# i2Nav-WHU/IC-GVINS

Hardware: AMD Instinct MI355X
Metric: frames/s at 1280x720, 300 feats, 10-KF window; residual/Jacobian eval/s (higher is better)
Workload: dtype u8/int64 front-end (f32/f64 solves), f64 factors

## Files before the change

ic-gvins_amd/csrc/detect.hip:

```cpp
#include <cfloat>

#include "icg_internal.h"


__device__ __forceinline__ unsigned int f32_order_key(float f) {
    unsigned int b = __float_as_uint(f);
    return (b & 0x80000000u) ? ~b : (b | 0x80000000u);
}
__device__ __forceinline__ float f32_from_order_key(unsigned int k) {
    unsigned int b = (k & 0x80000000u) ? (k & 0x7fffffffu) : ~k;
    return __uint_as_float(b);
}

#define FE_TW 60
#define FE_TH 16
#define FE_WAVES 4
#define FE_MAX_RADIUS 1022
#ifndef FE_RESIDENT_PER_XCD
#define FE_RESIDENT_PER_XCD 192
#endif

__device__ __forceinline__ float from_left(float v) {
    return __int_as_float(__builtin_amdgcn_mov_dpp(__float_as_int(v), 0x138, 0xF, 0xF, true));
}
__device__ __forceinline__ float from_right(float v) {
    return __int_as_float(__builtin_amdgcn_mov_dpp(__float_as_int(v), 0x130, 0xF, 0xF, true));
}

__device__ __forceinline__ unsigned int wave_or_to_lane63(unsigned int v) {
    v |= (unsigned int) __builtin_amdgcn_update_dpp(0, (int) v, 0xB1, 0xF, 0xF, false);
    v |= (unsigned int) __builtin_amdgcn_update_dpp(0, (int) v, 0x4E, 0xF, 0xF, false);
    v |= (unsigned int) __builtin_amdgcn_update_dpp(0, (int) v, 0x141, 0xF, 0xF, false);
    v |= (unsigned int) __builtin_amdgcn_update_dpp(0, (int) v, 0x140, 0xF, 0xF, false);
    v |= (unsigned int) __builtin_amdgcn_update_dpp(0, (int) v, 0x142, 0xA, 0xF, false);
    v |= (unsigned int) __builtin_amdgcn_update_dpp(0, (int) v, 0x143, 0xC, 0xF, false);
    return v;
}

#ifndef FE_CH
#define FE_CH 4
#endif
#define FE_GAP 6

__device__ __forceinline__ float fe_max(float a, float b) {
    float d;
    asm("v_max_f32 %0, %1, %2" : "=v"(d) : "v"(a), "v"(b));
    return d;
}

enum { FE_PLAIN = 0, FE_MIRRORS = 1, FE_PRIME = 2 };
struct fe_rows {
    int d0 = 0, d1 = 0, s0 = 0, s1 = 0;
    double hA0 = 0, hA1 = 0, hB0 = 0, hB1 = 0, hC0 = 0, hC1 = 0;
    float eC = 0.f, sideC = 0.f, m3T = 0.f, m3C = 0.f;
    bool unmC = false;
    float emax = -INFINITY;

    template <int MODE>
    __device__ __forceinline__ void chunk(unsigned int (&pix)[FE_CH], int y_last , const uint8_t *img,
                                          int base , int pitch, int ry, int h, unsigned int uc, int y0, int rh, int rw,
                                          unsigned int sel, float s, bool nms_col, int lane, int roi, int xcol, int32_t *cand_cnt,
                                          unsigned long long *cbase) {
        typedef unsigned int __attribute__((aligned(1))) u32u;
#pragma unroll
        for (int i = 0; i < FE_CH; i++) {
            const int y = y0 + i;
            const unsigned int v = __builtin_amdgcn_perm(0u, pix[i], sel);
            {
                const uint8_t *rowp = img + (size_t) icg_reflect1(min(max(ry + min(y + FE_CH, y_last), -1), h), h) * pitch;
                unsigned int vb = (unsigned int) base;
                asm("" : "+v"(vb));
                pix[i] = *reinterpret_cast<const u32u *>(rowp + vb);
            }
            const int a3 = (int) (v & 0xffu), b3 = (int) ((v >> 8) & 0xffu), c3 = (int) ((v >> 16) & 0xffu);
            const int dN = c3 - a3, sN = a3 + 2 * b3 + c3;
            if (MODE != FE_PRIME || i >= 2) {
                const int gxv = d0 + 2 * d1 + dN, gyv = sN - s0;
                const float dx = (float) gxv * s, dy = (float) gyv * s;
                const float cx = dx * dx, cm = dx * dy, cy = dy * dy;
                double hAn = ((double) from_left(cx) + (double) cx) + (double) from_right(cx);
                double hBn = ((double) from_left(cm) + (double) cm) + (double) from_right(cm);
                double hCn = ((double) from_left(cy) + (double) cy) + (double) from_right(cy);
                if (MODE != FE_PRIME) {
// ... 100 lines not shown
    }
    unsigned long long need;
    {
        unsigned int lo = (unsigned int) unmasked, hi = (unsigned int) (unmasked >> 32);
        lo = wave_or_to_lane63(lo);
        hi = wave_or_to_lane63(hi);
        need = ((unsigned long long) (unsigned int) __builtin_amdgcn_readlane((int) hi, 63) << 32) | (unsigned int) __builtin_amdgcn_readlane((int) lo, 63);
    }
    if (need == 0ull) return;
    typedef unsigned int __attribute__((aligned(1))) u32u;
    float emax = -INFINITY;
    while (need) {
        const int a = __ffsll((long long) need) - 1;
        unsigned long long closed = need;
#pragma unroll
        for (int g = 1; g <= FE_GAP; g++) closed |= need << g;
        const unsigned long long from_a = closed >> a;
        const int len                   = (~from_a == 0ull) ? 64 : __ffsll((long long) ~from_a) - 1;
        const unsigned long long runset = (len >= 64 ? ~0ull : ((1ull << len) - 1ull)) << a;
        const unsigned long long inrun  = need & runset;
        const int b                     = 63 - __builtin_clzll(inrun);
        need &= ~runset;
        const unsigned long long urun = (unmasked & inrun) >> a;
        const int y_first = by0 + a - 3, n_rows = b - a + 7;

        fe_rows st;
        st.emax = emax;
        unsigned int pix[FE_CH];
#pragma unroll
        for (int i = 0; i < FE_CH; i++) {
            const uint8_t *rowp = img + (size_t) icg_reflect1(min(max(R.ry + y_first + i, -1), h), h) * pitch;
            pix[i] = *reinterpret_cast<const u32u *>(rowp + (unsigned int) base);
        }
        const int y_last = y_first + n_rows - 1;
        st.chunk<FE_PRIME>(pix, y_last, img, base, pitch, R.ry, h, 0u, y_first, R.rh, R.rw, sel, s, nms_col, lane, roi, xcol, cand_cnt, cbase);
        for (int t0 = FE_CH; t0 < n_rows; t0 += FE_CH) {
            const unsigned int uc = t0 >= 5 ? (unsigned int) (urun >> (t0 - 5)) : (unsigned int) urun << (5 - t0);
            const int y0 = y_first + t0;
            if ((y0 <= 2 && 2 < y0 + FE_CH) || (y0 <= R.rh + 1 && R.rh + 1 < y0 + FE_CH))
                st.chunk<FE_MIRRORS>(pix, y_last, img, base, pitch, R.ry, h, uc, y0, R.rh, R.rw, sel, s, nms_col, lane, roi, xcol, cand_cnt, cbase);
            else
                st.chunk<FE_PLAIN>(pix, y_last, img, base, pitch, R.ry, h, uc, y0, R.rh, R.rw, sel, s, nms_col, lane, roi, xcol, cand_cnt, cbase);
        }
        emax = st.emax;
    }
    unsigned int key = emax == -INFINITY ? 0u : f32_order_key(emax);
#pragma unroll
    for (int m = 32; m >= 1; m >>= 1) {
        const unsigned int o = __shfl_xor(key, m, 64);
        key                  = o > key ? o : key;
    }
    if (lane == 0 && key) atomicMax(&roi_max[roi], key);
}

__global__ __launch_bounds__(64 * FE_WAVES) void k_min_eig_nms(const det_roi *rois, const uint8_t *frames, size_t slot_bytes,
                                                               const int32_t *slots, int pitch, int w, int h, const float2 *mask_pts,
                                                               const int32_t *mask_begin, const int32_t *mask_cnt , int radius,
                                                               const int32_t *vspan ,
                                                               unsigned int *roi_max,
                                                               unsigned long long *cand, size_t cand_plane, int32_t *cand_cnt,
                                                               int gx, int gy, int n_blocks, unsigned int m_roi, unsigned int m_gx) {
    __shared__ int vh[FE_MAX_RADIUS + 2];
    for (int a = threadIdx.x; a < radius + 2; a += 64 * FE_WAVES) vh[a] = vspan[a];
    __syncthreads();
    const int n_items = (n_blocks + FE_WAVES - 1) / FE_WAVES;
    const int chunk   = (n_items + 7) >> 3;
    const int x = blockIdx.x & 7, j = blockIdx.x >> 3, G = gridDim.x >> 3;
    const int wv  = __builtin_amdgcn_readfirstlane((int) (threadIdx.x >> 6));
    const int end = min((x + 1) * chunk, n_items);
    for (int it = x * chunk + j; it < end; it += G) {
        const int bl = it * FE_WAVES + wv;
        if (bl < n_blocks)
            fe_block(bl, vh, rois, frames, slot_bytes, slots, pitch, w, h, mask_pts, mask_begin, mask_cnt, radius, roi_max, cand, cand_plane, cand_cnt, gx, gy,
                     m_roi, m_gx);
    }
}

#define DET_MAX_PER_BLOCK 64

struct subpix_mask_t {
    float m[121];
};

struct subpix_smem {
    double terms[121][5];
    float patch[13][13];
    float cur[2];
    int stop;
};

#define DET_WAVE_SYNC()                                         \
    do {                                                        \
        __builtin_amdgcn_fence(__ATOMIC_SEQ_CST, "workgroup");  \
        __builtin_amdgcn_wave_barrier();                        \
    } while (0)

__device__ __forceinline__ float2 subpix_corner(subpix_smem &S, const det_roi &R, const uint8_t *img, int pitch, const float2 cT, int lane,
                                                const subpix_mask_t &M) {
    float cIx = cT.x, cIy = cT.y;
    int iter = 0;
    while (true) {
        const float ox = cIx - 6.f, oy = cIy - 6.f;
        const int iox = (int) floorf(ox), ioy = (int) floorf(oy);
        const float fa = ox - iox, fb = oy - ioy;
        const float w00 = (1.f - fa) * (1.f - fb), w01 = fa * (1.f - fb), w10 = (1.f - fa) * fb, w11 = fa * fb;
        for (int i = lane; i < 169; i += 64) {
            int r = i / 13, c = i - r * 13;
            int x0 = min(max(iox + c, 0), R.rw - 1), x1 = min(max(iox + c + 1, 0), R.rw - 1);
            int y0 = min(max(ioy + r, 0), R.rh - 1), y1 = min(max(ioy + r + 1, 0), R.rh - 1);
            const uint8_t *p0 = img + (size_t) (R.ry + y0) * pitch + R.rx;
            const uint8_t *p1 = img + (size_t) (R.ry + y1) * pitch + R.rx;
            float s00 = p0[x0], s01 = p0[x1], s10 = p1[x0], s11 = p1[x1];
            S.patch[r][c] = s00 * w00 + s01 * w01 + s10 * w10 + s11 * w11;
        }
        DET_WAVE_SYNC();
        for (int i = lane; i < 121; i += 64) {
            int r = i / 11, c = i - r * 11;
            double m   = M.m[i];
            double tgx = S.patch[r + 1][c + 2] - S.patch[r + 1][c];
            double tgy = S.patch[r + 2][c + 1] - S.patch[r][c + 1];
            double gxx = tgx * tgx * m, gxy = tgx * tgy * m, gyy = tgy * tgy * m;
            double px = c - 5, py = r - 5;
            S.terms[i][0] = gxx;
            S.terms[i][1] = gxy;
            S.terms[i][2] = gyy;
            S.terms[i][3] = gxx * px + gxy * py;
            S.terms[i][4] = gxy * px + gyy * py;
        }
        DET_WAVE_SYNC();
        double acc = 0;
        {
            const int q = lane % 5;
#pragma unroll 11
            for (int i = 0; i < 121; i++) acc += S.terms[i][q];
        }
        const double a = __shfl(acc, 0, 64), b = __shfl(acc, 1, 64), c = __shfl(acc, 2, 64);
        const double bb1 = __shfl(acc, 3, 64), bb2 = __shfl(acc, 4, 64);
        int st     = 0;
        float c2x = cIx, c2y = cIy;
        double det = a * c - b * b;
        if (fabs(det) <= DBL_EPSILON * DBL_EPSILON) {
            st = 1;
        } else {
            double scale = 1.0 / det;
            c2x          = (float) (cIx + c * scale * bb1 - b * scale * bb2);
            c2y          = (float) (cIy - b * scale * bb1 + a * scale * bb2);
            double err   = (double) ((c2x - cIx) * (c2x - cIx) + (c2y - cIy) * (c2y - cIy));
            if (c2x < 0 || c2x >= R.rw || c2y < 0 || c2y >= R.rh)
                st = 2;
            else if (!(iter + 1 < 20 && err > 0.01 * 0.01))
                st = 2;
        }
        if (st != 1) {
            cIx = c2x;
            cIy = c2y;
        }
        ++iter;
        DET_WAVE_SYNC();
        if (st) break;
    }
    if (fabsf(cIx - cT.x) > 5 || fabsf(cIy - cT.y) > 5) {
        cIx = cT.x;
        cIy = cT.y;
    }
    return make_float2(cIx, cIy);
}

__global__ __launch_bounds__(256) void k_select(const det_roi *rois, unsigned long long *cand, size_t cand_plane, int32_t *cand_cnt, unsigned int *roi_max,
                                                int min_dist, float2 *picks , int32_t *pick_cnt, int32_t *cnt_out, int max_pb) {
    __shared__ unsigned long long wbest[4];
    __shared__ unsigned long long best;
    const det_roi R = rois[blockIdx.x];
    const int t     = threadIdx.x;
    if (R.quota <= 0) {
        if (t == 0) pick_cnt[blockIdx.x] = 0, cnt_out[blockIdx.x] = 0;
        return;
    }
    unsigned long long *C = cand + (size_t) R.job * cand_plane + R.cand_base;
    const int n = cand_cnt[blockIdx.x];
    const double md2 = (double) min_dist * (double) min_dist;
    int quota = R.quota < max_pb ? R.quota : max_pb;
    int acc   = 0;
    {
        const unsigned int mk = roi_max[blockIdx.x];
        const double maxVal   = mk ? (double) f32_from_order_key(mk) : 0.0;
        const float thresh    = (float) (maxVal * 0.01);
        for (int i = t; i < n; i += 256)
            if (!(f32_from_order_key((unsigned int) (C[i] >> 32)) > thresh)) C[i] = 0;
        __syncthreads();
    }
    while (acc < quota) {
        unsigned long long k = 0;
        for (int i = t; i < n; i += 256) {
            unsigned long long c = C[i];
            k                    = c > k ? c : k;
        }
#pragma unroll
        for (int m = 32; m >= 1; m >>= 1) {
            unsigned long long o = __shfl_xor(k, m, 64);
            k                    = o > k ? o : k;
        }
        if ((t & 63) == 0) wbest[t >> 6] = k;
        __syncthreads();
        if (t == 0) {
            unsigned long long b = wbest[0];
            for (int i = 1; i < 4; i++) b = wbest[i] > b ? wbest[i] : b;
            best = b;
        }
        __syncthreads();
        const unsigned long long b = best;
        if (b == 0) break;
        const int idx = (int) (b & 0xffffffffu);
        const int by = idx / R.rw, bx = idx - by * R.rw;
        if (t == 0) picks[(size_t) blockIdx.x * max_pb + acc] = make_float2((float) bx, (float) by);
        acc++;
        if (min_dist >= 1) {
            for (int i = t; i < n; i += 256) {
                unsigned long long c = C[i];
                if (!c) continue;
                int ci = (int) (c & 0xffffffffu);
                int cy = ci / R.rw, cx = ci - cy * R.rw;
                float dx = (float) (cx - bx), dy = (float) (cy - by);
                if (c == b || (double) (dx * dx + dy * dy) < md2) C[i] = 0;
            }
        } else {
            for (int i = t; i < n; i += 256)
                if (C[i] == b) C[i] = 0;
        }
        __syncthreads();
    }
    if (t == 0) {
        pick_cnt[blockIdx.x] = acc;
        cnt_out[blockIdx.x]  = acc;
        roi_max[blockIdx.x]  = 0;
        cand_cnt[blockIdx.x] = 0;
    }
}

__global__ __launch_bounds__(64) void k_subpix(const det_roi *rois, const uint8_t *frames, size_t slot_bytes, const int32_t *slots, int pitch,
                                               const float2 *picks, float2 *corners_out, const int32_t *pick_cnt, int max_pb, subpix_mask_t M) {
    __shared__ subpix_smem SP;
    const int roi = blockIdx.x / max_pb, ci = blockIdx.x - roi * max_pb;
    if (ci >= pick_cnt[roi]) return;
    const det_roi R    = rois[roi];
    const uint8_t *img = frames + (size_t) slots[R.job] * slot_bytes;
    const float2 r     = subpix_corner(SP, R, img, pitch, picks[(size_t) roi * max_pb + ci], (int) threadIdx.x, M);
    if (threadIdx.x == 0) corners_out[(size_t) roi * max_pb + ci] = r;
}

static void circle_halfwidths(int radius, std::vector<int32_t> &hw) {
    hw.assign((size_t) radius + 1, -1);
    int err = 0, dx = radius, dy = 0, plus = 1, minus = (radius << 1) - 1;
    while (dx >= dy) {
        if (dx > hw[dy]) hw[dy] = dx;
        if (dy > hw[dx]) hw[dx] = dy;
        dy++;
        err += plus;
        plus += 2;
        int m = (err <= 0) - 1;
        err -= minus & m;
        dx += m;
        minus -= m & 2;
    }
}

static bool circle_row_spans(const std::vector<int32_t> &hw, std::vector<int32_t> &vh) {
    const int radius = (int) hw.size() - 1;
    vh.assign((size_t) radius + 2, -1);
    for (int a = 0; a <= radius; a++)
        for (int dy = 0; dy <= radius; dy++)
            if (hw[(size_t) dy] >= a) vh[(size_t) a] = dy;
    for (int a = 0; a <= radius; a++)
        for (int dy = 0; dy <= radius; dy++)
            if ((hw[(size_t) dy] >= a) != (dy <= vh[(size_t) a])) return false;
    return true;
}

static int ensure_roi_state(icg_ctx *ctx, int n_roi) {
    if (n_roi <= ctx->roi_state_cap) return 0;
    ICG_HIP(ctx, hipStreamSynchronize(ctx->stream));
    if (ctx->d_roi_max) (void) hipFree(ctx->d_roi_max);
    if (ctx->d_cand_cnt) (void) hipFree(ctx->d_cand_cnt);
    ctx->d_roi_max = nullptr, ctx->d_cand_cnt = nullptr, ctx->roi_state_cap = 0;
    const int cap = std::max(1024, 2 * n_roi);
    ICG_HIP(ctx, hipMalloc((void **) &ctx->d_roi_max, sizeof(uint32_t) * (size_t) cap));
    ICG_HIP(ctx, hipMalloc((void **) &ctx->d_cand_cnt, sizeof(int32_t) * (size_t) cap));
    ICG_HIP(ctx, hipMemsetAsync(ctx->d_roi_max, 0, sizeof(uint32_t) * (size_t) cap, ctx->stream));
    ICG_HIP(ctx, hipMemsetAsync(ctx->d_cand_cnt, 0, sizeof(int32_t) * (size_t) cap, ctx->stream));
    ctx->roi_state_cap = cap;
    return 0;
}

static subpix_mask_t subpix_window() {
    subpix_mask_t M;
    for (int i = 0; i < 11; i++) {
        float y  = (float) (i - 5) / 5;
        float vy = std::exp(-y * y);
        for (int j = 0; j < 11; j++) {
            float x         = (float) (j - 5) / 5;
            M.m[i * 11 + j] = (float) (vy * std::exp(-x * x));
        }
    }
    return M;
}

static int ensure_detect_ws(icg_ctx *ctx) {
    if (ctx->d_cand) return 0;
    const size_t w = ctx->cfg.width, h = ctx->cfg.height, nb = ctx->cfg.max_batch;
    ICG_HIP(ctx, hipMalloc((void **) &ctx->d_cand, sizeof(unsigned long long) * w * h * nb));
    return 0;
}

int icg_detect_check_grid(icg_ctx *ctx, const icg_detect_grid *grid) {
    if (grid->block_cols * grid->block_rows <= 0 || grid->block_w <= 6 || grid->block_h <= 6 || grid->block_cols * grid->block_w > ctx->cfg.width ||
        grid->block_rows * grid->block_h > ctx->cfg.height || grid->min_dist < 0 || grid->max_per_block <= 0 ||
        grid->max_per_block > DET_MAX_PER_BLOCK || grid->min_dist > FE_MAX_RADIUS)
        return icg_fail(ctx, ICG_ERR_INVALID, "bad detection grid");
    return 0;
}

static int detect_launch(icg_ctx *ctx, int n_roi, const icg_detect_grid *grid, const det_roi *d_rois, const int32_t *d_slots, const float2 *d_mask_pts,
                         const int32_t *d_mask_begin, const int32_t *d_mask_cnt, const int32_t *d_vh, float2 *d_picks, int32_t *d_pick_cnt,
                         float2 *d_corners, int32_t *d_corner_cnt) {
    const int w = ctx->cfg.width, h = ctx->cfg.height, pitch = ctx->lv[0].pitch, max_pb = grid->max_per_block;
    const size_t cand_plane = (size_t) w * h;
    {
        icg_prof_scope ps(ctx, "detect_min_eig_nms");
        const int gx = (grid->block_w + FE_TW - 1) / FE_TW, gy = (grid->block_h + FE_TH * FE_WAVES - 1) / (FE_TH * FE_WAVES);
        hipLaunchKernelGGL(k_min_eig_nms, dim3(std::min(icg_xcd_grid((gx * gy * n_roi + FE_WAVES - 1) / FE_WAVES), 8 * FE_RESIDENT_PER_XCD)), dim3(64 * FE_WAVES), 0, ctx->stream, d_rois, ctx->d_frames,
                           ctx->slot_bytes, d_slots, pitch, w, h, d_mask_pts, d_mask_begin, d_mask_cnt, grid->min_dist, d_vh, ctx->d_roi_max, ctx->d_cand,
                           cand_plane, ctx->d_cand_cnt, gx, gy, gx * gy * n_roi, icg_div_magic(gx * gy), icg_div_magic(gx));
    }
    {
        icg_prof_scope ps(ctx, "detect_select");
        hipLaunchKernelGGL(k_select, dim3(n_roi), dim3(256), 0, ctx->stream, d_rois, ctx->d_cand, cand_plane, ctx->d_cand_cnt, ctx->d_roi_max, grid->min_dist,
                           d_picks, d_pick_cnt, d_corner_cnt, max_pb);
    }
    {
        const subpix_mask_t M = subpix_window();
        icg_prof_scope ps(ctx, "detect_subpix");
        hipLaunchKernelGGL(k_subpix, dim3(n_roi * max_pb), dim3(64), 0, ctx->stream, d_rois, ctx->d_frames, ctx->slot_bytes, d_slots, pitch,
                           (const float2 *) d_picks, d_corners, (const int32_t *) d_pick_cnt, max_pb, M);
    }
    ICG_HIP(ctx, hipGetLastError());
    return ICG_OK;
}

extern "C" int icg_detect(icg_ctx *ctx, int n, const int32_t *slots, const icg_detect_grid *grid, const int32_t *mask_off,
                          const float *mask_pts, const int32_t *quota, int max_per_job, float *out_pts,
                          int32_t *out_count, int32_t *out_block) {
    if (!ctx || n < 0) return ICG_ERR_INVALID;
    if (n == 0) return ICG_OK;
    if (!slots || !grid || !mask_off || !quota || !out_pts || !out_count || max_per_job <= 0) return ICG_ERR_INVALID;
    if (n > ctx->cfg.max_batch) return icg_fail(ctx, ICG_ERR_CAPACITY, "detect batch %d > max_batch %d", n, ctx->cfg.max_batch);
    int rc = icg_detect_check_grid(ctx, grid);
    if (rc) return rc;
    const int nblk = grid->block_cols * grid->block_rows;
    for (int k = 0; k < n; k++)
        if (slots[k] < 0 || slots[k] >= ctx->cfg.n_slots) return icg_fail(ctx, ICG_ERR_INVALID, "bad slot");
    const int n_mask = mask_off[n];
    if (n_mask < 0 || (n_mask > 0 && !mask_pts)) return ICG_ERR_INVALID;
    ICG_HIP(ctx, hipSetDevice(ctx->cfg.device));
    if ((rc = ensure_detect_ws(ctx))) return rc;

    std::vector<det_roi> rois;
    for (int b = 0; b < n; b++)
        for (int k = 0; k < nblk; k++) {
            int q = quota[(size_t) b * nblk + k];
            if (q <= 0) continue;
            if (q > grid->max_per_block) q = grid->max_per_block;
            int cols = k % grid->block_cols, rows = k / grid->block_cols;
            det_roi R;
            R.job   = b;
            R.block = k;
            R.rx    = cols * grid->block_w;
            R.ry    = rows * grid->block_h;
            R.rw    = grid->block_w;
            R.rh    = grid->block_h;
            if (k != nblk - 1) {
                R.rw -= 5;
                R.rh -= 5;
            }
            R.quota     = q;
            R.cand_base = k * grid->block_w * grid->block_h;
            rois.push_back(R);
        }
    const int n_roi = (int) rois.size();
    for (int b = 0; b < n; b++) out_count[b] = 0;
    if (n_roi == 0) return ICG_OK;
    const int max_pb = grid->max_per_block;

    std::vector<int32_t> hw, vh;
    circle_halfwidths(grid->min_dist, hw);
    if (!circle_row_spans(hw, vh)) return icg_fail(ctx, ICG_ERR_INVALID, "circle span table of radius %d is not monotone", grid->min_dist);
    for (int b = 0; b < n; b++)
        if (mask_off[b] < 0 || mask_off[b] > mask_off[b + 1]) return icg_fail(ctx, ICG_ERR_INVALID, "mask_off is not non-decreasing");

    icg_call c(ctx);
    size_t need = sizeof(det_roi) * n_roi + sizeof(int32_t) * (2 * (size_t) n + 1 + vh.size()) + sizeof(float) * 2 * n_mask +
                  2 * (sizeof(float2) * max_pb + 16) * (size_t) n_roi + 8192;
    if ((rc = c.reserve(need))) return rc;
    const det_roi *d_rois  = c.in_zc(rois.data(), (size_t) n_roi);
    const int32_t *d_slots = c.in_zc(slots, (size_t) n);
    const int32_t *d_vh    = c.in(vh.data(), vh.size());
    const float2 *d_mpts   = (const float2 *) c.in(mask_pts, 2 * (size_t) n_mask);
    std::vector<int32_t> mcnt((size_t) n);
    for (int b = 0; b < n; b++) mcnt[(size_t) b] = mask_off[b + 1] - mask_off[b];
    const int32_t *d_moff  = c.in(mask_off, (size_t) n);
    const int32_t *d_mcnt  = c.in(mcnt.data(), (size_t) n);
    if ((rc = ensure_roi_state(ctx, n_roi))) return rc;
    if ((rc = c.seal())) return rc;
    std::vector<float> h_corners((size_t) n_roi * max_pb * 2);
    std::vector<int32_t> h_cnt((size_t) n_roi);
    float2 *d_picks = (float2 *) c.out((float *) nullptr, (size_t) n_roi * max_pb * 2);
    int32_t *d_pcnt = c.out((int32_t *) nullptr, (size_t) n_roi);
    float2 *z_corners  = (float2 *) c.out_zc(h_corners.data(), (size_t) n_roi * max_pb * 2);
    int32_t *z_cnt     = c.out_zc(h_cnt.data(), (size_t) n_roi);

    ICG_LAUNCH_GUARD(c);
    if ((rc = detect_launch(ctx, n_roi, grid, d_rois, d_slots, d_mpts, d_moff, d_mcnt, d_vh, d_picks, d_pcnt, z_corners, z_cnt))) return rc;
    if ((rc = c.finish())) return rc;

    for (int r = 0; r < n_roi; r++) {
        const det_roi &R = rois[r];
        for (int i = 0; i < h_cnt[r]; i++) {
// ... 31 lines not shown
```

ic-gvins_amd/csrc/lk.hip:

```cpp
#include <cfloat>

#include "dev_camera.h"
#include "icg_internal.h"

using namespace icgd;

#define LK_IT 24
#define LK_IS 28
#define LK_JT 32
#define LK_JS 36
#define LK_JM 5
#define LK_MAX_ITERS 30
#ifndef LK_WAVES_PER_EU
#define LK_WAVES_PER_EU 5
#endif

struct lk_smem {
    unsigned int I[LK_IT * LK_IS / 4];
    unsigned int J[LK_JT * LK_JS / 4 + 1];
};

__device__ __forceinline__ int dpp_add_xor1(int v) { return v + __builtin_amdgcn_update_dpp(0, v, 0xB1, 0xF, 0xF, false); }
__device__ __forceinline__ int dpp_add_xor2(int v) { return v + __builtin_amdgcn_update_dpp(0, v, 0x4E, 0xF, 0xF, false); }
__device__ __forceinline__ int dpp_add_half_mirror(int v) { return v + __builtin_amdgcn_update_dpp(0, v, 0x141, 0xF, 0xF, false); }
// ... 113 lines not shown
typedef unsigned int __attribute__((aligned(1))) lk_u32u;

__device__ __forceinline__ void lk_load_I(unsigned int (&v)[3], const unsigned char *I, int W, int H, int pitch, int ipx, int ipy,
                                          int lane) {
    const bool inside = ipx - 1 >= 0 && ipx - 1 + LK_IT <= W && ipy - 1 >= 0 && ipy - 1 + LK_IT <= H;
#pragma unroll
    for (int q = 0; q < 3; q++) {
        const int i = lane + 64 * q;
        const int r = i / 6, cd = i - r * 6;
        v[q] = 0;
        if (i < LK_IT * 6) {
            if (inside)
                v[q] = *reinterpret_cast<const lk_u32u *>(I + (size_t) (ipy - 1 + r) * pitch + (ipx - 1 + 4 * cd));
            else
                v[q] = lk_load4(I + (size_t) icg_reflect101(ipy - 1 + r, H) * pitch, ipx - 1 + 4 * cd, W);
        }
    }
}
__device__ __forceinline__ void lk_store_I(lk_smem &S, const unsigned int (&v)[3], int lane) {
#pragma unroll
    for (int q = 0; q < 3; q++) {
        const int i = lane + 64 * q;
        const int r = i / 6, cd = i - r * 6;
        if (i < LK_IT * 6) S.I[(r * LK_IS >> 2) + cd] = v[q];
    }
}
__device__ __forceinline__ void lk_load_J(unsigned int (&v)[4], const unsigned char *J, int W, int H, int pitch, int jx0, int jy0,
                                          int lane) {
    const int r = lane >> 1, c0 = (lane & 1) * 16;
    const bool inside = jx0 >= 0 && jx0 + LK_JT <= W && jy0 >= 0 && jy0 + LK_JT <= H;
    if (inside) {
        const unsigned char *row = J + (size_t) (jy0 + r) * pitch + (jx0 + c0);
#pragma unroll
        for (int q = 0; q < 4; q++) v[q] = *reinterpret_cast<const lk_u32u *>(row + 4 * q);
    } else {
        const unsigned char *row = J + (size_t) icg_reflect101(jy0 + r, H) * pitch;
#pragma unroll
        for (int q = 0; q < 4; q++) v[q] = lk_load4(row, jx0 + c0 + 4 * q, W);
    }
}
__device__ __forceinline__ void lk_store_J(lk_smem &S, const unsigned int (&v)[4], int lane) {
    const int r = lane >> 1, c0 = (lane & 1) * 16;
    unsigned int *dst = &S.J[(r * LK_JS + c0) >> 2];
#pragma unroll
    for (int q = 0; q < 4; q++) dst[q] = v[q];
}
__device__ __forceinline__ void lk_stage_J(lk_smem &S, const unsigned char *J, int W, int H, int pitch, int jx0, int jy0,
                                           int lane) {
    unsigned int v[4];
    lk_load_J(v, J, W, H, pitch, jx0, jy0, lane);
    lk_store_J(S, v, lane);
}

typedef short s16x2 __attribute__((ext_vector_type(2)));
typedef unsigned short u16x2 __attribute__((ext_vector_type(2)));

__device__ __forceinline__ unsigned int pk_add(unsigned int a, unsigned int b) {
    return __builtin_bit_cast(unsigned int, (u16x2) (__builtin_bit_cast(u16x2, a) + __builtin_bit_cast(u16x2, b)));
}
__device__ __forceinline__ unsigned int pk_sub(unsigned int a, unsigned int b) {
    return __builtin_bit_cast(unsigned int, (u16x2) (__builtin_bit_cast(u16x2, a) - __builtin_bit_cast(u16x2, b)));
}
__device__ __forceinline__ unsigned int pk_mul(unsigned int a, unsigned short k) {
    return __builtin_bit_cast(unsigned int, (u16x2) (__builtin_bit_cast(u16x2, a) * k));
}
__device__ __forceinline__ int dot2(unsigned int a, unsigned int b, int c) {
    return __builtin_amdgcn_sdot2(__builtin_bit_cast(s16x2, a), __builtin_bit_cast(s16x2, b), c, false);
}
__device__ __forceinline__ int dot2_keep(unsigned int a, unsigned int b, int c) {
    int d;
    asm("v_dot2_i32_i16 %0, %1, %2, %3" : "=v"(d) : "v"(a), "v"(b), "v"(c));
    return d;
}
__device__ __forceinline__ int dot2_keep_s(unsigned int a, unsigned int b, int c_uniform) {
    int d;
    asm("v_dot2_i32_i16 %0, %1, %2, %3" : "=v"(d) : "v"(a), "v"(b), "s"(c_uniform));
    return d;
}
__device__ __forceinline__ int dot2_zero(unsigned int a, unsigned int b) {
    int d;
    asm("v_dot2_i32_i16 %0, %1, %2, 0" : "=v"(d) : "v"(a), "v"(b));
    return d;
}
__device__ __forceinline__ unsigned int pk_lo16(int a, int b) {
    return __builtin_amdgcn_perm((unsigned int) b, (unsigned int) a, 0x05040100u);
}
__device__ __forceinline__ unsigned int pk_hi16(int a, int b) {
    return __builtin_amdgcn_perm((unsigned int) b, (unsigned int) a, 0x07060302u);
}
__device__ __forceinline__ unsigned int pk_shift(unsigned int a, unsigned int b) { return __builtin_amdgcn_alignbit(b, a, 16); }

__device__ __forceinline__ void lk_fetch_J(const lk_smem &S, int row0, int o, unsigned int (&JA)[7], unsigned int (&JB)[7]) {
    const int idx = o >> 2, sh = o & 3;
    const unsigned int *r0 = &S.J[(row0 * LK_JS >> 2) + idx];
    const unsigned int *r1 = r0 + (LK_JS >> 2);
    const unsigned int d0 = r0[0], d1 = r0[1], d2 = r0[2];
    const unsigned int e0 = r1[0], e1 = r1[1], e2 = r1[2];
    const unsigned int a0 = __builtin_amdgcn_alignbyte(d1, d0, sh), a1 = __builtin_amdgcn_alignbyte(d2, d1, sh);
    const unsigned int b0 = __builtin_amdgcn_alignbyte(e1, e0, sh), b1 = __builtin_amdgcn_alignbyte(e2, e1, sh);
#pragma unroll
    for (int k = 0; k < 7; k++) {
        const unsigned int sel = 0x0c000c00u | (unsigned int) k | ((unsigned int) (k + 1) << 16);
        JA[k] = __builtin_amdgcn_perm(a1, a0, sel);
        JB[k] = __builtin_amdgcn_perm(b1, b0, sel);
    }
}

__device__ bool lk_track_wave(const icg_pyr_desc &P, const unsigned char *slotI, const unsigned char *slotJ,
                              float2 prevPt, float2 &nextIO, lk_smem &S, int lane, float *err_out) {
    const float FLT_SCALE = 1.f / (1 << 20);
    const double eps2     = 0.01 * 0.01;
    bool status           = true;
    float errv            = 0.f;
    float2 nextStore      = nextIO;
    const int maxLevel    = P.n_levels - 1;
    const bool active     = lane < 63;
    const int ly          = active ? lane / 3 : 0;
    const int lx0         = active ? (lane - ly * 3) * 7 : 0;
    const unsigned int am = active ? ~0u : 0u;
    int rnd15 = 1 << 15, rnd8 = 1 << 8;
    asm volatile("" : "+s"(rnd15), "+s"(rnd8));

    for (int level = maxLevel; level >= 0; --level) {
        const int W = P.w[level], H = P.h[level], pitch = P.pitch[level];
        const unsigned char *I = slotI + P.off[level];
        const unsigned char *J = slotJ + P.off[level];
        const float scale      = (float) (1. / (1 << level));
        float prevx = prevPt.x * scale, prevy = prevPt.y * scale;
        float nptx, npty;
        if (level == maxLevel) {
            nptx = nextStore.x * scale;
            npty = nextStore.y * scale;
        } else {
            nptx = nextStore.x * 2.f;
            npty = nextStore.y * 2.f;
        }
        nextStore = make_float2(nptx, npty);

        prevx -= (float) ICG_LK_HALF;
        prevy -= (float) ICG_LK_HALF;
        const int ipx = (int) floorf(prevx), ipy = (int) floorf(prevy);
        if (ipx < -ICG_LK_WIN || ipx >= W || ipy < -ICG_LK_WIN || ipy >= H) {
            if (level == 0) {
                status = false;
                errv   = 0.f;
            }
            continue;
        }
        unsigned int W0, W1;
        lk_weights_pk(prevx - ipx, prevy - ipy, W0, W1);

        int jx0 = -1000000, jy0 = -1000000;
        {
            const int inx0 = (int) floorf(nptx - (float) ICG_LK_HALF), iny0 = (int) floorf(npty - (float) ICG_LK_HALF);
            const bool jok = !(inx0 < -ICG_LK_WIN || inx0 >= W || iny0 < -ICG_LK_WIN || iny0 >= H);
            unsigned int vi[3] = {0, 0, 0}, vj[4] = {0, 0, 0, 0};
            lk_load_I(vi, I, W, H, pitch, ipx, ipy, lane);
            if (jok) {
                jx0 = inx0 - LK_JM;
                jy0 = iny0 - LK_JM;
                lk_load_J(vj, J, W, H, pitch, jx0, jy0, lane);
            }
            __syncthreads();
            lk_store_I(S, vi, lane);
            if (jok) lk_store_J(S, vj, lane);
            __syncthreads();
        }

        int c0[7];
        unsigned int IXP[4], IYP[4];
        int sA11 = 0, sA12 = 0, sA22 = 0;
        float A11, A12, A22;
        {
            const int idx = lx0 >> 2, sh = lx0 & 3;
            unsigned int Pp[4][5];
            const unsigned int sel0 = 0x0c000c00u | (unsigned int) sh | ((unsigned int) (sh + 1) << 16), sel1 = sel0 + 0x00020002u;
#pragma unroll
            for (int r = 0; r < 4; r++) {
                const unsigned int *p = &S.I[((ly + r) * LK_IS >> 2) + idx];
                const unsigned int d0 = p[0], d1 = p[1], d2 = p[2], d3 = p[3];
                Pp[r][0] = __builtin_amdgcn_perm(d1, d0, sel0);
                Pp[r][1] = __builtin_amdgcn_perm(d1, d0, sel1);
                Pp[r][2] = __builtin_amdgcn_perm(d2, d1, sel0);
                Pp[r][3] = __builtin_amdgcn_perm(d2, d1, sel1);
                Pp[r][4] = __builtin_amdgcn_perm(d3, d2, sel0);
            }
            const bool all_in = ipx >= 0 && ipx + 22 <= W && ipy >= 0 && ipy + 22 <= H;
            unsigned int DX[2][4], DY[2][4];
#pragma unroll
            for (int rr = 0; rr < 2; rr++) {
                unsigned int T0[5], T1[5];
#pragma unroll
                for (int m = 0; m < 5; m++) {
                    T0[m] = pk_add(pk_mul(pk_add(Pp[rr][m], Pp[rr + 2][m]), 12), pk_mul(Pp[rr + 1][m], 40));
                    T1[m] = pk_sub(Pp[rr + 2][m], Pp[rr][m]);
                }
#pragma unroll
                for (int m = 0; m < 4; m++) {
                    DX[rr][m] = pk_sub(T0[m + 1], T0[m]);
                    DY[rr][m] = pk_add(pk_mul(pk_add(T1[m], T1[m + 1]), 12), pk_mul(pk_shift(T1[m], T1[m + 1]), 40));
                }
            }
            if (!all_in) {
                asm volatile("" ::: "memory");
#pragma unroll
                for (int rr = 0; rr < 2; rr++) {
                    const int Y           = ipy + ly + rr;
                    const unsigned int RM = (Y >= 0 && Y < H) ? ~0u : 0u;
#pragma unroll
                    for (int m = 0; m < 4; m++) {
                        const int X0 = ipx + lx0 + 2 * m, X1 = X0 + 1;
                        const unsigned int CM = ((X0 >= 0 && X0 < W) ? 0x0000ffffu : 0u) | ((X1 >= 0 && X1 < W) ? 0xffff0000u : 0u);
                        DX[rr][m] &= CM & RM;
                        DY[rr][m] &= CM & RM;
                    }
                }
            }
            int bx[7], by[7];
            const unsigned int W0d = W0 & am, W1d = W1 & am;
#pragma unroll
            for (int k = 0; k < 7; k++) {
                const int m = k >> 1;
                const unsigned int dx0 = (k & 1) ? pk_shift(DX[0][m], DX[0][m + 1]) : DX[0][m];
                const unsigned int dx1 = (k & 1) ? pk_shift(DX[1][m], DX[1][m + 1]) : DX[1][m];
                const unsigned int dy0 = (k & 1) ? pk_shift(DY[0][m], DY[0][m + 1]) : DY[0][m];
                const unsigned int dy1 = (k & 1) ? pk_shift(DY[1][m], DY[1][m + 1]) : DY[1][m];
                const int m1 = (k + 1) >> 1;
                const unsigned int i1 = ((k + 1) & 1) ? pk_shift(Pp[1][m1], Pp[1][m1 + 1]) : Pp[1][m1];
                const unsigned int i2 = ((k + 1) & 1) ? pk_shift(Pp[2][m1], Pp[2][m1 + 1]) : Pp[2][m1];
                bx[k]        = dot2(dx1, W1d, dot2_keep_s(dx0, W0d, rnd15));
                by[k]        = dot2(dy1, W1d, dot2_keep_s(dy0, W0d, rnd15));
                c0[k]        = 256 - (dot2(i2, W1, dot2_keep_s(i1, W0, rnd8)) & ~511);
            }
#pragma unroll
            for (int m = 0; m < 4; m++) {
                IXP[m] = m < 3 ? pk_hi16(bx[2 * m], bx[2 * m + 1]) : (unsigned int) bx[6] >> 16;
                IYP[m] = m < 3 ? pk_hi16(by[2 * m], by[2 * m + 1]) : (unsigned int) by[6] >> 16;
            }
            sA11 = dot2(IXP[3], IXP[3], dot2(IXP[2], IXP[2], dot2(IXP[1], IXP[1], dot2(IXP[0], IXP[0], 0))));
            sA12 = dot2(IXP[3], IYP[3], dot2(IXP[2], IYP[2], dot2(IXP[1], IYP[1], dot2(IXP[0], IYP[0], 0))));
            sA22 = dot2(IYP[3], IYP[3], dot2(IYP[2], IYP[2], dot2(IYP[1], IYP[1], dot2(IYP[0], IYP[0], 0))));
            wave_sum3_i32x16_f32(sA11, sA12, sA22, A11, A12, A22);
            A11 *= FLT_SCALE, A12 *= FLT_SCALE, A22 *= FLT_SCALE;
        }
        float D            = A11 * A22 - A12 * A12;
        const float eig2 = A22 + A11 - icg_sqrt_unscaled((A11 - A22) * (A11 - A22) + 4.f * A12 * A12);
        static_assert(ICG_LK_WIN == 21, "the threshold constant below is for a 21 x 21 window");
        const bool weak = eig2 < __uint_as_float(0x3DB4A233u) || D < FLT_EPSILON;
        if (weak) {
            if (level == 0) status = false;
            continue;
        }
        D = 1.f / D;
        const float Ds = D * FLT_SCALE;
        nptx -= (float) ICG_LK_HALF;
        npty -= (float) ICG_LK_HALF;
        float pdx = 0.f, pdy = 0.f;
        int cinx = -1000000, ciny = -1000000;
        unsigned int JA[7], JB[7];
#pragma unroll
        for (int k = 0; k < 7; k++) JA[k] = JB[k] = 0;

        int j = 0;
        bool more = true;
        while (more) {
            const float fx = floorf(nptx), fy = floorf(npty);
            const int inx = (int) fx, iny = (int) fy;
            if (inx < -ICG_LK_WIN || inx >= W || iny < -ICG_LK_WIN || iny >= H) {
                if (level == 0) status = false;
                break;
            }
            if (!(inx >= jx0 && inx <= jx0 + (LK_JT - 22) && iny >= jy0 && iny <= jy0 + (LK_JT - 22))) {
                jx0 = inx - LK_JM;
                jy0 = iny - LK_JM;
                __syncthreads();
                lk_stage_J(S, J, W, H, pitch, jx0, jy0, lane);
                __syncthreads();
            }
            lk_fetch_J(S, iny - jy0 + ly, (inx - jx0) + lx0, JA, JB);
            cinx = inx;
            ciny = iny;
            float ax = nptx - fx, ay = npty - fy;
            for (;;) {
                lk_weights_pk(ax, ay, W0, W1);
                int diff[7];
#pragma unroll
                for (int k = 0; k < 7; k++) diff[k] = dot2(JB[k], W1, dot2_keep(JA[k], W0, c0[k])) >> 9;
                int sb1 = 0, sb2 = 0;
#pragma unroll
                for (int m = 0; m < 4; m++) {
                    const unsigned int dp = m < 3 ? pk_lo16(diff[2 * m], diff[2 * m + 1]) : (unsigned int) diff[6];
                    sb1 = m ? dot2(dp, IXP[m], sb1) : dot2_zero(dp, IXP[m]);
                    sb2 = m ? dot2(dp, IYP[m], sb2) : dot2_zero(dp, IYP[m]);
                }
                float b1, b2;
                wave_sum2_i32x8_f32(sb1, sb2, b1, b2);
                const float dx = (float) ((A12 * b2 - A22 * b1) * Ds);
                const float dy = (float) ((A12 * b1 - A11 * b2) * Ds);
                nptx += dx;
                npty += dy;
                nextStore = make_float2(nptx + (float) ICG_LK_HALF, npty + (float) ICG_LK_HALF);
                const float n2 = dx * dx + dy * dy;
                bool converged = n2 < 9.9999e-5f;
                if (!converged && !(n2 > 1.00001e-4f)) {
                    asm volatile("");
                    converged = __builtin_fma((double) dx, (double) dx, (double) dy * (double) dy) <= eps2;
                }
                if (converged) {
                    more = false;
                    break;
                }
                if (j > 0 && fabsf(dx + pdx) <= 0.01f && fabsf(dy + pdy) <= 0.01f) {
                    nextStore.x -= dx * 0.5f;
                    nextStore.y -= dy * 0.5f;
                    more = false;
                    break;
                }
                pdx = dx;
                pdy = dy;
                if (++j >= LK_MAX_ITERS) {
                    more = false;
                    break;
                }
                ax = nptx - fx;
                ay = npty - fy;
                if (!(__float_as_uint(ax) < 0x3f800000u && __float_as_uint(ay) < 0x3f800000u)) break;
            }
        }

        if (status && level == 0) {
            const float ex = nextStore.x - (float) ICG_LK_HALF, ey = nextStore.y - (float) ICG_LK_HALF;
            const int inx = (int) floorf(ex), iny = (int) floorf(ey);
            if (inx < -ICG_LK_WIN || inx >= W || iny < -ICG_LK_WIN || iny >= H) {
                status = false;
                continue;
            }
            if (err_out) {
                if (inx != cinx || iny != ciny) {
                    if (!(inx >= jx0 && inx <= jx0 + (LK_JT - 22) && iny >= jy0 && iny <= jy0 + (LK_JT - 22))) {
                        jx0 = inx - LK_JM;
                        jy0 = iny - LK_JM;
                        __syncthreads();
                        lk_stage_J(S, J, W, H, pitch, jx0, jy0, lane);
                        __syncthreads();
                    }
                    lk_fetch_J(S, iny - jy0 + ly, (inx - jx0) + lx0, JA, JB);
                }
                lk_weights_pk(ex - inx, ey - iny, W0, W1);
                int se = 0;
#pragma unroll
                for (int k = 0; k < 7; k++) {
                    const int diff = dot2(JB[k], W1, dot2_keep(JA[k], W0, c0[k])) >> 9;
                    se += diff < 0 ? -diff : diff;
                }
                se &= (int) am;
                errv = wave_sum_i32x16_f32(se) * 1.f / (float) (32 * ICG_LK_WIN * ICG_LK_WIN);
            }
        }
    }
    nextIO = nextStore;
    if (err_out && lane == 0) *err_out = errv;
    return status;
}

__global__ __launch_bounds__(64) void k_lk_track(icg_pyr_desc P, int n, const int32_t *prev_slot, const int32_t *next_slot,
                                                 const float2 *prev_pts, float2 *next_pts, unsigned char *status, float *err) {
    __shared__ lk_smem S;
    const int i = icg_xcd_chunked(blockIdx.x, n);
    if (i >= n) return;
    const int lane = threadIdx.x;
    const unsigned char *sI = P.base + (size_t) prev_slot[i] * P.slot_bytes;
    const unsigned char *sJ = P.base + (size_t) next_slot[i] * P.slot_bytes;
    float2 nx = next_pts[i];
    bool st   = lk_track_wave(P, sI, sJ, prev_pts[i], nx, S, lane, err ? err + i : nullptr);
    if (lane == 0) {
        next_pts[i] = nx;
        status[i]   = st ? 1 : 0;
    }
}

__global__ __launch_bounds__(64, LK_WAVES_PER_EU) void k_lk_track_fb(icg_pyr_desc P, int n, const int32_t *prev_slot,
                                                    const int32_t *next_slot, const float2 *prev_pts,
                                                    const float2 *guess_pts, float2 *out_pts, unsigned char *status,
                                                    float2 *out_bwd, int img_w, int img_h,
                                                    int seg_cap, const int32_t *seg_count) {
    __shared__ lk_smem S;
    const int i = icg_xcd_chunked(blockIdx.x, n);
    if (i >= n) return;
    if (seg_count) {
        const int s = i / seg_cap;
        if (i - s * seg_cap >= seg_count[s]) return;
    }
    const int lane = threadIdx.x;
    const unsigned char *sP = P.base + (size_t) prev_slot[i] * P.slot_bytes;
    const unsigned char *sN = P.base + (size_t) next_slot[i] * P.slot_bytes;
    const float2 p0 = prev_pts[i];
    float2 fwd      = guess_pts[i];
    float2 bwd      = p0;
    bool st_f = false, st_b = false;
    for (int dir = 0; dir < 2; dir++) {
        if (dir) {
            const bool border = fwd.x < 5.f || fwd.y < 5.f || fwd.x > (float) (img_w - 5) || fwd.y > (float) (img_h - 5);
            if (!st_f || border) break;
        }
        const unsigned char *a = dir ? sN : sP, *b = dir ? sP : sN;
        const float2 from      = dir ? fwd : p0;
        float2 io              = dir ? bwd : fwd;
        const bool st          = lk_track_wave(P, a, b, from, io, S, lane, nullptr);
        if (dir) {
            bwd  = io;
            st_b = st;
        } else {
            fwd  = io;
            st_f = st;
        }
    }
    if (lane == 0) {
        out_pts[i] = fwd;
        out_bwd[i] = bwd;
        status[i]  = (unsigned char) ((st_f && st_b) ? 1u : 0u);
    }
}

__global__ __launch_bounds__(256) void k_lk_finish(int n, const float2 *prev_pts, const float2 *out_pts, float2 *bwd_undist, unsigned char *status,
                                                   int want_undist, int has_cam, icg_camera cam, int img_w, int img_h, int seg_cap,
                                                   const int32_t *seg_count) {
    const int i = blockIdx.x * 256 + threadIdx.x;
    if (i >= n) return;
    if (seg_count) {
        const int s = i / seg_cap;
        if (i - s * seg_cap >= seg_count[s]) return;
    }
    const float2 p0 = prev_pts[i], fwd = out_pts[i], bwd = bwd_undist[i];
    const bool border = (double) fwd.x < 5.0 || (double) fwd.y < 5.0 || ((double) fwd.x > (img_w - 5.0)) || ((double) fwd.y > (img_h - 5.0));
    const double ddx = (double) (bwd.x - p0.x), ddy = (double) (bwd.y - p0.y);
// ... 125 lines not shown
```

Measured before the change: 159,000.

## Pack four subpixel corners per wave and fold LK diff shifts into operands

The subpixel refinement kernel now handles four corners per 64-lane wave, 16 lanes each. It caches the raw 14x14 integer patch and reloads it only when the integer origin moves, uses ds_swizzle row broadcasts in place of full-wave shuffles, and exits once a ballot shows every corner frozen. Separately, the LK tracker pre-scales the J packs and c0 constants by 128. This lets the high half of each dot2 accumulator serve as the packed diff directly, which removes the per-element shift and pk_lo16 repack in the inner Gauss-Newton loop. The changes add precision and overflow risk in the 16-bit fixed-point path, and converged lanes idle while they wait for slower corners.

New measurement: 132,200. -16.8%, worse.

```diff
diff --git a/ic-gvins_amd/csrc/detect.hip b/ic-gvins_amd/csrc/detect.hip
--- a/ic-gvins_amd/csrc/detect.hip
+++ b/ic-gvins_amd/csrc/detect.hip
@@ -1,4 +1,5 @@
 #include <cfloat>
+#include <climits>
 
 #include "icg_internal.h"
 
@@ -265,11 +266,12 @@
     float m[121];
 };
 
+#define SUBPIX_PACK 4
+
 struct subpix_smem {
-    double terms[121][5];
-    float patch[13][13];
-    float cur[2];
-    int stop;
+    double terms[121][SUBPIX_PACK][5];
+    float patch[SUBPIX_PACK][13][13];
+    float raw[SUBPIX_PACK][14][14];
 };
 
 #define DET_WAVE_SYNC()                                         \
@@ -278,47 +280,63 @@
         __builtin_amdgcn_wave_barrier();                        \
     } while (0)
 
-__device__ __forceinline__ float2 subpix_corner(subpix_smem &S, const det_roi &R, const uint8_t *img, int pitch, const float2 cT, int lane,
-                                                const subpix_mask_t &M) {
+template <int Q>
+__device__ __forceinline__ double subpix_row_bcast(double v) {
+    int lo = __double2loint(v), hi = __double2hiint(v);
+    lo     = __builtin_amdgcn_ds_swizzle(lo, 0x10 | (Q << 5));
+    hi     = __builtin_amdgcn_ds_swizzle(hi, 0x10 | (Q << 5));
+    return __hiloint2double(hi, lo);
+}
+
+__device__ __forceinline__ float2 subpix_corners(subpix_smem &S, const det_roi &R, const uint8_t *img, int pitch, const float2 cT, bool live, int lane,
+                                                 const subpix_mask_t &M) {
+    const int l = lane & 15, cn = lane >> 4;
     float cIx = cT.x, cIy = cT.y;
-    int iter = 0;
+    int kx = INT_MIN, ky = INT_MIN;
+    bool frozen = !live;
+    int iter    = 0;
     while (true) {
         const float ox = cIx - 6.f, oy = cIy - 6.f;
         const int iox = (int) floorf(ox), ioy = (int) floorf(oy);
         const float fa = ox - iox, fb = oy - ioy;
         const float w00 = (1.f - fa) * (1.f - fb), w01 = fa * (1.f - fb), w10 = (1.f - fa) * fb, w11 = fa * fb;
-        for (int i = lane; i < 169; i += 64) {
-            int r = i / 13, c = i - r * 13;
-            int x0 = min(max(iox + c, 0), R.rw - 1), x1 = min(max(iox + c + 1, 0), R.rw - 1);
-            int y0 = min(max(ioy + r, 0), R.rh - 1), y1 = min(max(ioy + r + 1, 0), R.rh - 1);
-            const uint8_t *p0 = img + (size_t) (R.ry + y0) * pitch + R.rx;
-            const uint8_t *p1 = img + (size_t) (R.ry + y1) * pitch + R.rx;
-            float s00 = p0[x0], s01 = p0[x1], s10 = p1[x0], s11 = p1[x1];
-            S.patch[r][c] = s00 * w00 + s01 * w01 + s10 * w10 + s11 * w11;
+        if (iox != kx || ioy != ky) {
+            for (int i = l; i < 196; i += 16) {
+                const int r = i / 14, c = i - r * 14;
+                const int x = min(max(iox + c, 0), R.rw - 1), y = min(max(ioy + r, 0), R.rh - 1);
+                S.raw[cn][r][c] = img[(size_t) (R.ry + y) * pitch + R.rx + x];
+            }
+            kx = iox, ky = ioy;
         }
         DET_WAVE_SYNC();
-        for (int i = lane; i < 121; i += 64) {
-            int r = i / 11, c = i - r * 11;
+        for (int i = l; i < 169; i += 16) {
+            const int r = i / 13, c = i - r * 13;
+            const float s00 = S.raw[cn][r][c], s01 = S.raw[cn][r][c + 1], s10 = S.raw[cn][r + 1][c], s11 = S.raw[cn][r + 1][c + 1];
+            S.patch[cn][r][c] = s00 * w00 + s01 * w01 + s10 * w10 + s11 * w11;
+        }
+        DET_WAVE_SYNC();
+        for (int i = l; i < 121; i += 16) {
+            const int r = i / 11, c = i - r * 11;
             double m   = M.m[i];
-            double tgx = S.patch[r + 1][c + 2] - S.patch[r + 1][c];
-            double tgy = S.patch[r + 2][c + 1] - S.patch[r][c + 1];
+            double tgx = S.patch[cn][r + 1][c + 2] - S.patch[cn][r + 1][c];
+            double tgy = S.patch[cn][r + 2][c + 1] - S.patch[cn][r][c + 1];
             double gxx = tgx * tgx * m, gxy = tgx * tgy * m, gyy = tgy * tgy * m;
             double px = c - 5, py = r - 5;
-            S.terms[i][0] = gxx;
-            S.terms[i][1] = gxy;
-            S.terms[i][2] = gyy;
-            S.terms[i][3] = gxx * px + gxy * py;
-            S.terms[i][4] = gxy * px + gyy * py;
+            S.terms[i][cn][0] = gxx;
+            S.terms[i][cn][1] = gxy;
+            S.terms[i][cn][2] = gyy;
+            S.terms[i][cn][3] = gxx * px + gxy * py;
+            S.terms[i][cn][4] = gxy * px + gyy * py;
         }
         DET_WAVE_SYNC();
         double acc = 0;
         {
-            const int q = lane % 5;
+            const int q = l % 5;
 #pragma unroll 11
-            for (int i = 0; i < 121; i++) acc += S.terms[i][q];
-        }
-        const double a = __shfl(acc, 0, 64), b = __shfl(acc, 1, 64), c = __shfl(acc, 2, 64);
-        const double bb1 = __shfl(acc, 3, 64), bb2 = __shfl(acc, 4, 64);
+            for (int i = 0; i < 121; i++) acc += S.terms[i][cn][q];
+        }
+        const double a = subpix_row_bcast<0>(acc), b = subpix_row_bcast<1>(acc), c = subpix_row_bcast<2>(acc);
+        const double bb1 = subpix_row_bcast<3>(acc), bb2 = subpix_row_bcast<4>(acc);
         int st     = 0;
         float c2x = cIx, c2y = cIy;
         double det = a * c - b * b;
@@ -334,13 +352,16 @@
             else if (!(iter + 1 < 20 && err > 0.01 * 0.01))
                 st = 2;
         }
-        if (st != 1) {
-            cIx = c2x;
-            cIy = c2y;
+        if (!frozen) {
+            if (st != 1) {
+                cIx = c2x;
+                cIy = c2y;
+            }
+            if (st) frozen = true;
         }
         ++iter;
         DET_WAVE_SYNC();
-        if (st) break;
+        if (__builtin_amdgcn_ballot_w64(!frozen) == 0) break;
     }
     if (fabsf(cIx - cT.x) > 5 || fabsf(cIy - cT.y) > 5) {
         cIx = cT.x;
@@ -421,14 +442,18 @@
 }
 
 __global__ __launch_bounds__(64) void k_subpix(const det_roi *rois, const uint8_t *frames, size_t slot_bytes, const int32_t *slots, int pitch,
-                                               const float2 *picks, float2 *corners_out, const int32_t *pick_cnt, int max_pb, subpix_mask_t M) {
+                                               const float2 *picks, float2 *corners_out, const int32_t *pick_cnt, int max_pb, int groups, subpix_mask_t M) {
     __shared__ subpix_smem SP;
-    const int roi = blockIdx.x / max_pb, ci = blockIdx.x - roi * max_pb;
-    if (ci >= pick_cnt[roi]) return;
+    const int roi = blockIdx.x / groups, ci0 = (blockIdx.x - roi * groups) * SUBPIX_PACK;
+    const int cnt = pick_cnt[roi];
+    if (ci0 >= cnt) return;
     const det_roi R    = rois[roi];
     const uint8_t *img = frames + (size_t) slots[R.job] * slot_bytes;
-    const float2 r     = subpix_corner(SP, R, img, pitch, picks[(size_t) roi * max_pb + ci], (int) threadIdx.x, M);
-    if (threadIdx.x == 0) corners_out[(size_t) roi * max_pb + ci] = r;
+    const int ci       = ci0 + ((int) threadIdx.x >> 4);
+    const bool live    = ci < cnt;
+    const float2 cT    = live ? picks[(size_t) roi * max_pb + ci] : make_float2(0.f, 0.f);
+    const float2 r     = subpix_corners(SP, R, img, pitch, cT, live, (int) threadIdx.x, M);
+    if (live && (threadIdx.x & 15) == 0) corners_out[(size_t) roi * max_pb + ci] = r;
 }
 
 static void circle_halfwidths(int radius, std::vector<int32_t> &hw) {
@@ -522,8 +547,9 @@
     {
         const subpix_mask_t M = subpix_window();
         icg_prof_scope ps(ctx, "detect_subpix");
-        hipLaunchKernelGGL(k_subpix, dim3(n_roi * max_pb), dim3(64), 0, ctx->stream, d_rois, ctx->d_frames, ctx->slot_bytes, d_slots, pitch,
-                           (const float2 *) d_picks, d_corners, (const int32_t *) d_pick_cnt, max_pb, M);
+        const int groups = (max_pb + SUBPIX_PACK - 1) / SUBPIX_PACK;
+        hipLaunchKernelGGL(k_subpix, dim3(n_roi * groups), dim3(64), 0, ctx->stream, d_rois, ctx->d_frames, ctx->slot_bytes, d_slots, pitch,
+                           (const float2 *) d_picks, d_corners, (const int32_t *) d_pick_cnt, max_pb, groups, M);
     }
     ICG_HIP(ctx, hipGetLastError());
     return ICG_OK;
diff --git a/ic-gvins_amd/csrc/lk.hip b/ic-gvins_amd/csrc/lk.hip
--- a/ic-gvins_amd/csrc/lk.hip
+++ b/ic-gvins_amd/csrc/lk.hip
@@ -219,9 +219,6 @@
     asm("v_dot2_i32_i16 %0, %1, %2, 0" : "=v"(d) : "v"(a), "v"(b));
     return d;
 }
-__device__ __forceinline__ unsigned int pk_lo16(int a, int b) {
-    return __builtin_amdgcn_perm((unsigned int) b, (unsigned int) a, 0x05040100u);
-}
 __device__ __forceinline__ unsigned int pk_hi16(int a, int b) {
     return __builtin_amdgcn_perm((unsigned int) b, (unsigned int) a, 0x07060302u);
 }
@@ -238,8 +235,8 @@
 #pragma unroll
     for (int k = 0; k < 7; k++) {
         const unsigned int sel = 0x0c000c00u | (unsigned int) k | ((unsigned int) (k + 1) << 16);
-        JA[k] = __builtin_amdgcn_perm(a1, a0, sel);
-        JB[k] = __builtin_amdgcn_perm(b1, b0, sel);
+        JA[k] = __builtin_amdgcn_perm(a1, a0, sel) << 7;
+        JB[k] = __builtin_amdgcn_perm(b1, b0, sel) << 7;
     }
 }
 
@@ -367,12 +364,12 @@
                 const unsigned int i2 = ((k + 1) & 1) ? pk_shift(Pp[2][m1], Pp[2][m1 + 1]) : Pp[2][m1];
                 bx[k]        = dot2(dx1, W1d, dot2_keep_s(dx0, W0d, rnd15));
                 by[k]        = dot2(dy1, W1d, dot2_keep_s(dy0, W0d, rnd15));
-                c0[k]        = 256 - (dot2(i2, W1, dot2_keep_s(i1, W0, rnd8)) & ~511);
+                c0[k]        = (256 - (dot2(i2, W1, dot2_keep_s(i1, W0, rnd8)) & ~511)) * 128;
             }
 #pragma unroll
             for (int m = 0; m < 4; m++) {
-                IXP[m] = m < 3 ? pk_hi16(bx[2 * m], bx[2 * m + 1]) : (unsigned int) bx[6] >> 16;
-                IYP[m] = m < 3 ? pk_hi16(by[2 * m], by[2 * m + 1]) : (unsigned int) by[6] >> 16;
+                IXP[m] = m < 3 ? pk_hi16(bx[2 * m], bx[2 * m + 1]) : (unsigned int) bx[6] & 0xffff0000u;
+                IYP[m] = m < 3 ? pk_hi16(by[2 * m], by[2 * m + 1]) : (unsigned int) by[6] & 0xffff0000u;
             }
             sA11 = dot2(IXP[3], IXP[3], dot2(IXP[2], IXP[2], dot2(IXP[1], IXP[1], dot2(IXP[0], IXP[0], 0))));
             sA12 = dot2(IXP[3], IYP[3], dot2(IXP[2], IYP[2], dot2(IXP[1], IYP[1], dot2(IXP[0], IYP[0], 0))));
@@ -420,13 +417,13 @@
             float ax = nptx - fx, ay = npty - fy;
             for (;;) {
                 lk_weights_pk(ax, ay, W0, W1);
-                int diff[7];
-#pragma unroll
-                for (int k = 0; k < 7; k++) diff[k] = dot2(JB[k], W1, dot2_keep(JA[k], W0, c0[k])) >> 9;
+                int acc[7];
+#pragma unroll
+                for (int k = 0; k < 7; k++) acc[k] = dot2(JB[k], W1, dot2_keep(JA[k], W0, c0[k]));
                 int sb1 = 0, sb2 = 0;
 #pragma unroll
                 for (int m = 0; m < 4; m++) {
-                    const unsigned int dp = m < 3 ? pk_lo16(diff[2 * m], diff[2 * m + 1]) : (unsigned int) diff[6];
+                    const unsigned int dp = m < 3 ? pk_hi16(acc[2 * m], acc[2 * m + 1]) : (unsigned int) acc[6];
                     sb1 = m ? dot2(dp, IXP[m], sb1) : dot2_zero(dp, IXP[m]);
                     sb2 = m ? dot2(dp, IYP[m], sb2) : dot2_zero(dp, IYP[m]);
                 }
@@ -487,7 +484,7 @@
                 int se = 0;
 #pragma unroll
                 for (int k = 0; k < 7; k++) {
-                    const int diff = dot2(JB[k], W1, dot2_keep(JA[k], W0, c0[k])) >> 9;
+                    const int diff = dot2(JB[k], W1, dot2_keep(JA[k], W0, c0[k])) >> 16;
                     se += diff < 0 ? -diff : diff;
                 }
                 se &= (int) am;
```
